# vita-epfl/CrowdNav

Measured on AMD Instinct MI355X. Metric: env-steps/sec (whole node), 4096 envs x 5 humans, ORCA step, higher is better.
Workload: dtype f32 ORCA solve + f64 env step

## Files before the change

### crowdnav_amd/csrc/rollout_fused.h

```cpp
#pragma once
#include "step_kernels.h"

namespace cn {

constexpr int kFusedMaxNC = 5;

template <typename T>
__device__ __forceinline__ T in_vgpr(T x) {
    asm volatile("" : "+v"(x));
    return x;
}

__device__ __forceinline__ void stage_agent(const Params& P, const Smem& s, const Lane& L, const AgentRegs& r,
                                            double human_safety) {
    if (L.lane >= P.nA) return;
    s.kin[L.lane] = make_float4((float)r.px, (float)r.py, (float)r.vx, (float)r.vy);
    s.posd[L.lane] = make_double2(r.px, r.py);
    s.rad[L.lane] = r.rad;
    s.hview[L.lane] = (float)(r.rad + 0.01 + human_safety);
}

__device__ __forceinline__ void preferred_velocity(const AgentRegs& r, float max_speed, bool solve, float4& sol, float4& start) {
    const double gdx = r.gx - r.px, gdy = r.gy - r.py;
    const double speed = norm2(gdx, gdy);
    const float pref_x = (float)(speed > 1.0 ? gdx / speed : gdx);
    const float pref_y = (float)(speed > 1.0 ? gdy / speed : gdy);
    sol = make_float4(pref_x, pref_y, max_speed, solve ? 1.0f : 0.0f);
    float sx, sy;
    lp_start_point(max_speed, pref_x, pref_y, sx, sy);
    start = make_float4(sx, sy, 0.0f, 0.0f);
}

#define CN_FUSED_SYNC() wave_lds_sync()



struct PairRow {
    int my_info, my_slot;
    unsigned long long row_slots;
};
__device__ __forceinline__ PairRow pair_row_of(const Params& P, const Smem& s, int lane) {
    PairRow pr{0, P.nA, 0ull};
    if (lane < P.pairs) {
        pr.my_info = s.pinfo[lane];
        const int c = (pr.my_info >> 16) & 0xff;
        for (int k = 0; k < kFusedMaxNC; ++k) {
            int slot = P.nA;
            if (k < P.NC) {
                const int ik = s.pinfo[lane - c + k];
                slot = ((ik >> 24) & 1) ? ((ik >> 8) & 0xff) : P.nA;
            }
            pr.row_slots |= (unsigned long long)slot << (8 * k);
        }
        pr.my_slot = (int)((pr.row_slots >> (8 * c)) & 0xffull);
    }
    return pr;
}

template <typename Mid>
__device__ __forceinline__ void fused_pair_phase(const Params& P, const Smem& s, const PairRow& pr, float range_sq, Mid&& mid) {
    const int my_info = pr.my_info, my_slot = pr.my_slot;
    const unsigned long long row_slots = pr.row_slots;
    const int q = my_info & 0xff, c = (my_info >> 16) & 0xff;
    const int ol = (my_info >> 8) & 0xff;
    const bool robot_sim = (my_info >> 25) & 1;
    const float4 me = s.kin[q];
    const float4 other = s.kin[my_slot];
    float4 ot[kFusedMaxNC];
#pragma unroll
    for (int k = 0; k < kFusedMaxNC; ++k) ot[k] = s.kin[(int)((row_slots >> (8 * k)) & 0xffull)];
    const float* view = robot_sim ? s.rview : s.hview;
    const float rsum = view[q] + view[ol];
    const float odx = me.x - other.x, ody = me.y - other.y;
    const float mine = odx * odx + ody * ody;
    int rank = 0, within = 0;
    {
        const uint32_t mb = __float_as_uint(mine), rb = __float_as_uint(range_sq);
        uint32_t before = 0u, inside = 0u;
#pragma unroll
        for (int k = 0; k < kFusedMaxNC; ++k) {
            const float dx = me.x - ot[k].x, dy = me.y - ot[k].y;
            const uint32_t vb = __float_as_uint(dx * dx + dy * dy);
            const uint32_t tie = (uint32_t)(k - c) >> 31;
            before = __builtin_amdgcn_alignbit(before, vb - mb - tie, 31);
            inside = __builtin_amdgcn_alignbit(inside, vb - rb, 31);
        }
        within = __popc(inside);
        rank = __popc(before & inside);
    }
    mid();
    if (c == 0) s.count[q] = within < P.orca.max_neighbors ? within : P.orca.max_neighbors;
    if (mine < range_sq && rank < P.orca.max_neighbors)
        s.lines[q * kLineStride + rank] =
            make_half_plane(P.orca, me.x, me.y, me.z, me.w, other.x, other.y, other.z, other.w, rsum);
}

template <int MAXL>
__device__ __forceinline__ void fused_candidates(const Params& P, const Smem& s, int lane) {
    if (lane < P.nA * MAXL) {
        const int q = lane / MAXL, k = lane - q * MAXL;
        const float4 so = s.sol[q];
        const float4* lq = s.lines + q * kLineStride;
        s.cand2[q * kLineStride + k] = lp_line_candidate_pairs5(lq, k, lane, so.z, so.x, so.y);
    }
}

__device__ __forceinline__ void split_barrier() {
    asm volatile("s_waitcnt lgkmcnt(0)\n\ts_barrier" ::: "memory");
}

struct Lp3Item {
    int a, m, i, base;
    bool item;
    float4 li, lj;
    float radius;
};
template <int MAXL>
__device__ __forceinline__ Lp3Item lp3_item_of(const Smem& s, int lane, unsigned long long mask) {
    constexpr int kPairs = MAXL * (MAXL - 1) / 2;
    Lp3Item it;
    const int t = lane / kPairs;
    it.m = lane - t * kPairs;
    it.a = 0;
    unsigned long long rest = mask;
#pragma unroll
    for (int u = 0; u < kWave / kPairs; ++u) {
        const int bit = rest ? __ffsll((long long)rest) - 1 : 0;
        it.a = (u == t) ? bit : it.a;
        rest &= rest - 1ull;
    }
    it.item = lane < (int)__popcll(mask) * kPairs;
    it.i = lp3_program_of(it.m), it.base = it.i * (it.i - 1) / 2;
    const float4* la = s.lines + it.a * kLineStride;
    it.li = la[it.i], it.lj = la[it.m - it.base];
    it.radius = s.sol[it.a].z;
    return it;
}
template <int MAXL>
__device__ __forceinline__ void lp3_head(const Smem& s, const Lp3Item& it) {
    const float4 pr = lp3_project(it.li, it.lj);
    if (it.item) s.proj[it.a * kLineStride + it.m] = pr;
    CN_FUSED_SYNC();
    if (it.item) {
        const float4* pa = s.proj + it.a * kLineStride + it.base;
        s.cand3[it.a * kLineStride + it.m] =
            lp_line_candidate<MAXL - 2>(pa[it.m - it.base], pa, it.m - it.base, it.radius, -it.li.w, it.li.z, true);
    }
}

template <int MAXL>
__device__ __forceinline__ bool split_has_head(unsigned int pred, int u, int n_steps) {
    return pred != 0u && __popc(pred) * (MAXL * (MAXL - 1) / 2) <= kWave && u < n_steps;
}

struct NoOp {
    __device__ __forceinline__ void operator()() const {}
};
template <int MAXL, int BASE_PRIO = 0, typename AfterScan = NoOp>
__device__ __forceinline__ unsigned long long fused_solve(const Params& P, const Smem& s, int lane, bool solve, float& rx,
                                                          float& ry, PhaseClock* clk, unsigned long long have = 0ull,
                                                          AfterScan&& after_scan = NoOp{}) {
    (void)P, (void)clk;
    rx = 0.0f, ry = 0.0f;
    int n = 0, fail = 0;
    if (solve) {
        n = s.count[lane];
        const float4 start = s.res[lane];
        rx = start.x, ry = start.y;
        fail = lp_planar_scan<MAXL>(s.lines + lane * kLineStride, s.cand2 + lane * kLineStride, n, rx, ry);
    }
    CN_TICK(clk, 3);
    const bool need = solve && fail < n;
    const unsigned long long nm = __ballot(need);
#ifdef CN_PHASE_TIMING
    if (clk) clk->acc[9] += __popcll(nm);
#endif
    after_scan();
    if (nm == 0ull) __builtin_amdgcn_s_setprio(BASE_PRIO);
    if (nm != 0ull) {
        __builtin_amdgcn_s_setprio(3);
        constexpr int kPairs = MAXL * (MAXL - 1) / 2;
        const int n_todo = __popcll(nm);
        bool one_pass_done = false;
        if (n_todo * kPairs <= kWave) {
            const Lp3Item it = lp3_item_of<MAXL>(s, lane, nm);
            const bool item = it.item;
            const int a = it.a, i = it.i, m = it.m, base = it.base;
            const float4 li = it.li;
            const float radius = it.radius;
            const bool hit = (nm & ~have) == 0ull;
            if (!hit) {
                lp3_head<MAXL>(s, it);
                CN_FUSED_SYNC();
            }
            if (item && m == base)
                s.cand2[a * kLineStride + i] = lp3_inner_program(s.proj + a * kLineStride, s.cand3 + a * kLineStride, i, li, radius);
            CN_FUSED_SYNC();
            if (need)
                lp3_outer_scan(s.lines + lane * kLineStride, s.cand2 + lane * kLineStride, n, fail, s.sol[lane].z, rx, ry);
            one_pass_done = true;
        } else {
            if (need) s.todo[__popcll(nm & ((1ull << lane) - 1ull))] = lane;
            CN_FUSED_SYNC();
            const int items = n_todo * kPairs;
            for (int p = lane; p < items; p += kWave) {
                const int t = p / kPairs, m = p - t * kPairs;
                const int a = s.todo[t];
                const int i = lp3_program_of(m), j = m - i * (i - 1) / 2;
                const float4* la = s.lines + a * kLineStride;
                s.proj[a * kLineStride + m] = lp3_project(la[i], la[j]);
            }
            CN_FUSED_SYNC();
            for (int p = lane; p < items; p += kWave) {
                const int t = p / kPairs, m = p - t * kPairs;
                const int a = s.todo[t];
                const int i = lp3_program_of(m), base = i * (i - 1) / 2;
                const float4 li = s.lines[a * kLineStride + i];
                const float4* pa = s.proj + a * kLineStride + base;
                s.cand3[a * kLineStride + m] = lp_line_candidate<MAXL - 2>(pa[m - base], pa, m - base, s.sol[a].z, -li.w, li.z, true);
            }
            CN_FUSED_SYNC();
        }
        if (need && !one_pass_done)
            lp3_scan(s.lines + lane * kLineStride, s.proj + lane * kLineStride, s.cand3 + lane * kLineStride, n,
                     fail, s.sol[lane].z, rx, ry);
    }
    return nm;
}

struct StepConsts {
    double dt, limit, limit1, success, collision, ddist, dfactor, hsafety;
};
__device__ __forceinline__ StepConsts step_consts(const Params& P) {
    StepConsts K;
    K.dt = in_vgpr(P.dt), K.limit = in_vgpr(P.time_limit), K.limit1 = in_vgpr(P.time_limit - 1.0);
    K.success = in_vgpr(P.success_reward), K.collision = in_vgpr(P.collision_penalty);
    K.ddist = in_vgpr(P.discomfort_dist), K.dfactor = in_vgpr(P.discomfort_factor);
    K.hsafety = in_vgpr(P.human_safety);
    return K;
}

__device__ __forceinline__ double swept_distance(const AgentRegs& r, bool human, double2 rp, double act_x, double act_y,
                                                 double new_vx, double new_vy, double dt, double robot_rad) {
    const double x1 = r.px - rp.x, y1 = r.py - rp.y;
    const double wx = r.vx - act_x, wy = r.vy - act_y;
    const double x2 = x1 + wx * dt, y2 = y1 + wy * dt;
    const double sx = x2 - x1, sy = y2 - y1;
    double u = ((0.0 - x1) * sx + (0.0 - y1) * sy) / (sx * sx + sy * sy);
    u = (u > 1.0) ? 1.0 : ((u < 0.0) ? 0.0 : u);
    const bool degenerate = (sx == 0.0 && sy == 0.0);
    const double cx = degenerate ? 0.0 - x1 : (x1 + u * sx) - 0.0;
    const double cy = degenerate ? 0.0 - y1 : (y1 + u * sy) - 0.0;
    const double endx = r.px + new_vx * dt, endy = r.py + new_vy * dt;
    const double d = norm2(human ? cx : endx - r.gx, human ? cy : endy - r.gy);
    return human ? d - r.rad - robot_rad : d;
}

struct StepOutcome {
    double reward, dmin;
    int info;
    bool done;
};
__device__ __forceinline__ StepOutcome reduce_env(const Params& P, const Smem& s, int ebase, double gtime, const StepConsts& K) {
    const double goal_dist = s.closest[ebase];
    const double robot_rad = s.rad[ebase];
    double dmin = std::numeric_limits<double>::infinity();
    bool collision = false;
    for (int i = 1; i < P.A; ++i) {
        const double c = s.closest[ebase + i];
        const bool hit = c < 0.0;
        dmin = (!collision & !hit & (c < dmin)) ? c : dmin;
        collision = collision | hit;
    }
    const bool timeout = gtime >= K.limit1;
    const bool reaching = goal_dist < robot_rad;
    const bool danger = dmin < K.ddist;
    double reward = danger ? (dmin - K.ddist) * K.dfactor * K.dt : 0.0;
    int info = danger ? CN_DANGER : CN_NOTHING;
    reward = reaching ? K.success : reward, info = reaching ? CN_REACH_GOAL : info;
    reward = collision ? K.collision : reward, info = collision ? CN_COLLISION : info;
    reward = timeout ? 0.0 : reward, info = timeout ? CN_TIMEOUT : info;
    const bool done = timeout | collision | reaching;
    return StepOutcome{reward, dmin, info, done};
}


#ifdef CN_WAVE_TRACE
static __device__ unsigned long long cn_wave_trace[8192 * 6];
#endif

constexpr int kSplitOrcaPrio = 1;
constexpr int kAssistHead = 1;
#ifndef CN_SPLIT_HEAD_PRIO
#define CN_SPLIT_HEAD_PRIO 2
#endif
#ifndef CN_SPLIT_HEAD_TAIL_PRIO
#define CN_SPLIT_HEAD_TAIL_PRIO 1
#endif

#ifdef CN_SPLIT_PROBE
constexpr bool kSplitProbe = true;
static __device__ unsigned long long cn_split_probe[32];
#define SPLIT_PROBE_DECL()                                                                                   \
    unsigned long long sp_cnt[7] = {}, sp_wait[3] = {}, sp_w1[2] = {}, sp_n1[2] = {}, sp_dt = 0ull; \
    bool sp_prev_head = false
#define SPLIT_PROBE_WAIT(k, barrier)                                   \
    do {                                                               \
        const unsigned long long sp_t0 = __builtin_readcyclecounter(); \
        barrier;                                                       \
        sp_dt = __builtin_readcyclecounter() - sp_t0;                  \
        sp_wait[k] += sp_dt;                                           \
    } while (0)
#define SPLIT_PROBE_AFTER_1(word, head)                               \
    do {                                                               \
        if ((word) != 0u) sp_w1[0] += sp_dt, ++sp_n1[0];               \
        if (sp_prev_head) sp_w1[1] += sp_dt, ++sp_n1[1];               \
        sp_prev_head = (head);                                         \
    } while (0)
#define SPLIT_PROBE_STEP(ended, nm, head, pred)                                  \
    do {                                                                         \
        const bool sp_hit = (head) && (nm) != 0ull && ((nm) & ~(unsigned long long)(pred)) == 0ull; \
        ++sp_cnt[0], sp_cnt[1] += (ended) ? 1 : 0, sp_cnt[2] += (nm) != 0ull ? 1 : 0, sp_cnt[3] += (head) ? 1 : 0; \
        sp_cnt[4] += sp_hit ? 1 : 0, sp_cnt[5] += ((nm) != 0ull && !sp_hit) ? 1 : 0, sp_cnt[6] += ((head) && (nm) == 0ull) ? 1 : 0; \
    } while (0)
#define SPLIT_PROBE_FLUSH(lane, base)                                                        \
    do {                                                                                     \
        if ((lane) == 0) {                                                                   \
            if ((base) == 0)                                                                 \
                for (int k = 0; k < 7; ++k) atomicAdd(&cn_split_probe[k], sp_cnt[k]);        \
            for (int k = 0; k < 3; ++k) atomicAdd(&cn_split_probe[((base) ? 10 : 7) + k], sp_wait[k]); \
            for (int k = 0; k < 2; ++k) {                                                    \
                atomicAdd(&cn_split_probe[((base) ? 17 : 13) + k], sp_w1[k]);                \
                atomicAdd(&cn_split_probe[((base) ? 19 : 15) + k], sp_n1[k]);                \
            }                                                                                \
        }                                                                                    \
    } while (0)
#else
constexpr bool kSplitProbe = false;
#define SPLIT_PROBE_DECL() (void)0
#define SPLIT_PROBE_WAIT(k, barrier) barrier
#define SPLIT_PROBE_AFTER_1(word, head) (void)0
#define SPLIT_PROBE_STEP(ended, nm, head, pred) (void)0
#define SPLIT_PROBE_FLUSH(lane, base) (void)0
#endif

template <int MAXL, int ASSIST>
__device__ __forceinline__ void split_orca_wave(const Params& P, const Smem& s, int n_steps) {
    const int lane = (int)threadIdx.x - kWave;
    float2* const vel = reinterpret_cast<float2*>(s.act);
    const float range_sq = P.orca.neighbor_dist * P.orca.neighbor_dist;
    const double c_dt = in_vgpr(P.dt);
    split_barrier();
    __builtin_amdgcn_s_setprio(kSplitOrcaPrio);
    const PairRow pr = pair_row_of(P, s, lane);
    double px = 0.0, py = 0.0;
    float rx = 0.0f, ry = 0.0f;
    bool solved = false;
    SPLIT_PROBE_DECL();
    for (int u = 0;;) {
        SPLIT_PROBE_WAIT(0, split_barrier());
        const bool ended = __builtin_amdgcn_readfirstlane(s.flag[0]) != 0;
        const unsigned int pred = ((ASSIST & kAssistHead) || kSplitProbe) ? (unsigned int)__builtin_amdgcn_readfirstlane(s.flag[1]) : 0u;
        if (!ended) ++u;
        if (u >= n_steps) {
            split_barrier();
            break;
        }
        const bool head = (ASSIST & kAssistHead) ? split_has_head<MAXL>(pred, u, n_steps) : false;
        SPLIT_PROBE_AFTER_1(pred, head);
        if (lane < P.nA) {
            if (ended) {
                const double2 p = s.posd[lane];
                px = p.x, py = p.y;
            } else if (solved) {
                px = px + (double)rx * c_dt;
                py = py + (double)ry * c_dt;
                s.kin[lane] = make_float4((float)px, (float)py, rx, ry);
            }
        }
        CN_FUSED_SYNC();
        if (lane < P.pairs) fused_pair_phase(P, s, pr, range_sq, [] {});
        SPLIT_PROBE_WAIT(1, split_barrier());
        fused_candidates<MAXL>(P, s, lane);
        CN_FUSED_SYNC();
        solved = lane < P.nA && s.sol[lane < P.nA ? lane : 0].w != 0.0f;
        const unsigned long long nm = fused_solve<MAXL, kSplitOrcaPrio>(P, s, lane, solved, rx, ry, nullptr, head ? pred : 0u, [&] {
            if (head) SPLIT_PROBE_WAIT(2, split_barrier());
        });
        if (lane < P.nA) vel[lane] = make_float2(rx, ry);
        if (((ASSIST & kAssistHead) || kSplitProbe) && lane == 0) s.flag[1] = (int)nm;
        SPLIT_PROBE_STEP(ended, nm, head, pred);
    }
    SPLIT_PROBE_FLUSH(lane, 0);
}

template <bool HEADLINE, bool SPLIT = false, int ASSIST = 0>
__global__ __launch_bounds__((SPLIT ? 2 : 1) * kWave, (SPLIT ? 4 : HEADLINE ? 3 : 1)) void rollout_fused_kernel(
    Params P_in, const StateView* Sd, const int* ring_filled_in, RolloutView R, int n_steps, const double* ext_action) {
    static_assert(HEADLINE || !SPLIT, "the two-wave kernel exists for the headline geometry only");
    static_assert(SPLIT || ASSIST == 0, "the env wave assists an ORCA wave: two-wave kernel only");
#ifdef CN_WAVE_TRACE
    const unsigned long long wt_entry = __builtin_amdgcn_s_memrealtime();
    unsigned long long wt_fallbacks = 0ull, wt_ends = 0ull;
#endif
    constexpr int MAXL = 5;
    Params P = P_in;
    P.async_fill = 0;
    if (HEADLINE) {
        P.A = 6, P.NC = 5, P.E = 2, P.nA = 12, P.pairs = 60, P.threads = 64;
    }
    const Smem s = carve<MAXL>(P);
    if constexpr (SPLIT) {
        if (__builtin_amdgcn_readfirstlane((int)threadIdx.x) >= kWave) {
            split_orca_wave<MAXL, ASSIST>(P, s, n_steps);
            return;
        }
    }
    const Lane L = lane_of(P);
    AgentRegs r = {};
    float robot_max_speed = 0.0f;
    const bool robot = L.valid && L.a == 0;
    const cn_rollout_io* iop = R.io;
    double theta = 0.0;
    EpisodeBook ep = {};
    {
        const StateView S = *Sd;
        const cn_rollout_io io = *iop;
        const size_t gi = L.valid ? L.gi : 0;
        const int env = L.valid ? L.env : 0;
        const double2 p0 = S.pos[gi], v0 = S.vel[gi], g0 = S.goal[gi], q0 = S.rv[gi];
        const bool have = P.robot_orca ? S.rsim_valid[env] != 0 : false;
        const float rr_kept = P.robot_orca ? S.rsim_radius[gi] : 0.0f;
        const float ms_kept = P.robot_orca ? S.rsim_max_speed[env] : 0.0f;
        const double theta0 = S.theta[env];
        EpisodeBook ep0;
        CN_LOAD_EPISODE(ep0, S, io, ring_filled_in, env);
        if (L.valid) {
            r.px = p0.x, r.py = p0.y, r.vx = v0.x, r.vy = v0.y, r.gx = g0.x, r.gy = g0.y, r.rad = q0.x, r.vpref = q0.y;
            ep = ep0;
            if (L.a == 0) theta = theta0;
            if (P.robot_orca) {
                const float rr = have ? rr_kept : (float)(r.rad + 0.01 + P.robot_safety);
                if (!have) S.rsim_radius[L.gi] = rr;
                s.rview[L.lane] = rr;
                if (L.a == 0) {
                    robot_max_speed = have ? ms_kept : (float)r.vpref;
                    if (!have) S.rsim_max_speed[L.env] = robot_max_speed;
                }
            }
        }
    }
    build_pairs(P, s);

    if (L.valid && ep.state == kWaitingScenario && scenario_ready(P, *Sd, L.env, ep.ep_count, ep.ring_filled)) {
        load_from_ring(P, *Sd, L, ep.ep_count % P.ring_depth, r);
        ep.state = kRunning;
        ep.gtime = 0.0;
        theta = 1.5707963267948966;
    }
    unsigned int transitions = 0;
    for (int t = threadIdx.x; t < kMaxDiscount; t += P.threads) s.disc[t] = t < R.discount_len ? R.discount[t] : 0.0;
    CN_FUSED_SYNC();
    if (L.lane == 0) s.kin[P.nA] = make_float4(std::numeric_limits<float>::infinity(), std::numeric_limits<float>::infinity(), 0.0f, 0.0f);
    const PairRow pr = pair_row_of(P, s, L.lane);
    const StepConsts K = step_consts(P);
    stage_agent(P, s, L, r, K.hsafety);
    CN_FUSED_SYNC();

#ifdef CN_PHASE_TIMING
    PhaseClock clock = {};
    PhaseClock* clk = &clock;
    clock.last = __builtin_readcyclecounter();
#else
    PhaseClock* clk = nullptr;
    (void)clk;
#endif
    const float range_sq = P.orca.neighbor_dist * P.orca.neighbor_dist;
#ifdef CN_WAVE_TRACE
    const unsigned long long wt_loop = __builtin_amdgcn_s_memrealtime();
#endif
    if constexpr (SPLIT) {
        float2* const vel = reinterpret_cast<float2*>(s.act);
        if (L.lane == 0) s.flag[0] = 1, s.flag[1] = 0;
        split_barrier();
        bool skip = true;
        SPLIT_PROBE_DECL();
        for (int u = 0;;) {
            SPLIT_PROBE_WAIT(0, split_barrier());
            if (!skip) ++u;
            const unsigned int pred = ((ASSIST & kAssistHead) || kSplitProbe) ? (unsigned int)__builtin_amdgcn_readfirstlane(s.flag[1]) : 0u;
            SPLIT_PROBE_AFTER_1(pred, (ASSIST & kAssistHead) != 0 && split_has_head<MAXL>(pred, u, n_steps));
            const bool running = L.valid && ep.state == kRunning;
            const AgentRegs r0 = r;
            double act_x = 0.0, act_y = 0.0, new_vx = 0.0, new_vy = 0.0;
            if (!skip && L.lane < P.nA) {
                const float2 mine = vel[L.lane], robots = vel[L.ebase];
                act_x = (double)robots.x, act_y = (double)robots.y;
                new_vx = (L.a == 0) ? act_x : (double)mine.x;
                new_vy = (L.a == 0) ? act_y : (double)mine.y;
                if (running) {
                    r.px = r.px + new_vx * K.dt;
                    r.py = r.py + new_vy * K.dt;
                    r.vx = new_vx;
                    r.vy = new_vy;
                }
            }
            if (u < n_steps && L.lane < P.nA) {
                float4 sol4, start4;
                preferred_velocity(r, (L.a == 0) ? robot_max_speed : (float)r.vpref, running && (L.a > 0 || P.robot_orca), sol4, start4);
                s.sol[L.lane] = sol4;
                s.res[L.lane] = start4;
            }
            SPLIT_PROBE_WAIT(1, split_barrier());
            if constexpr ((ASSIST & kAssistHead) != 0) {
                if (split_has_head<MAXL>(pred, u, n_steps)) {
                    __builtin_amdgcn_s_setprio(CN_SPLIT_HEAD_PRIO);
                    const Lp3Item it = lp3_item_of<MAXL>(s, L.lane, (unsigned long long)pred);
                    lp3_head<MAXL>(s, it);
                    __builtin_amdgcn_s_setprio(CN_SPLIT_HEAD_TAIL_PRIO);
                    SPLIT_PROBE_WAIT(2, split_barrier());
                }
            }
            bool ended = false;
            if (!skip) {
                const double2 rp = make_double2(__shfl(r0.px, L.ebase), __shfl(r0.py, L.ebase));
                if (L.valid) s.closest[L.lane] = swept_distance(r0, L.a > 0, rp, act_x, act_y, new_vx, new_vy, K.dt, s.rad[L.ebase]);
                CN_FUSED_SYNC();
                bool done = false;
                if (running) {
                    const double disc_t = s.disc[ep.cur_steps < kMaxDiscount ? ep.cur_steps : kMaxDiscount - 1];
                    const StepOutcome o = reduce_env(P, s, L.ebase, ep.gtime, K);
                    done = o.done;
                    ep.gtime += K.dt;
                    ++transitions;
                    CN_BOOK_TRANSITION(ep, ep.cur_steps < kMaxDiscount ? disc_t : 0.0, o.reward, o.info, o.dmin);
                    if (done) {
                        const cn_rollout_io io = *iop;
                        const StateView S = *Sd;
                        AgentRegs next = r;
                        load_from_ring(P, S, L, (ep.ep_count + 1) % P.ring_depth, next);
                        CN_END_EPISODE(P, S, io, L.env, L.a == 0, K.limit, o.info, ep, r = next; theta = 1.5707963267948966);
                    }
                }
                ended = __ballot(done) != 0ull;
            }
            if (ended) stage_agent(P, s, L, r, K.hsafety);
            if (L.lane == 0) s.flag[0] = ended ? 1 : 0;
            skip = ended;
            if constexpr ((ASSIST & kAssistHead) != 0 && CN_SPLIT_HEAD_TAIL_PRIO != 0) __builtin_amdgcn_s_setprio(0);
            if (u >= n_steps) break;
        }
        SPLIT_PROBE_FLUSH(L.lane, 10);
    }
    const int one_wave_steps = SPLIT ? 0 : n_steps;
    for (int step = 0; step < one_wave_steps; ++step) {
        const bool running = L.valid && ep.state == kRunning;
        const bool solve = running && (L.a > 0 || P.robot_orca);

        if (L.lane < P.pairs) {
            float4 sol4, start4;
            fused_pair_phase(P, s, pr, range_sq, [&] {
                preferred_velocity(r, (L.a == 0) ? robot_max_speed : (float)r.vpref, solve, sol4, start4);
            });
            if (L.lane < P.nA) {
                s.sol[L.lane] = sol4;
                s.res[L.lane] = start4;
            }
        }
        CN_FUSED_SYNC();
        CN_TICK(clk, 2);

        fused_candidates<MAXL>(P, s, L.lane);
        CN_FUSED_SYNC();

        float rx, ry;
        const bool fell_back = fused_solve<MAXL>(P, s, L.lane, solve, rx, ry, clk) != 0ull;
        (void)fell_back;
#ifdef CN_WAVE_TRACE
        if (fell_back) ++wt_fallbacks;
#endif
        CN_TICK(clk, 8);

        double act_x, act_y;
        if (P.robot_orca) {
            act_x = (double)__shfl(rx, L.ebase);
            act_y = (double)__shfl(ry, L.ebase);
        } else {
            act_x = L.valid ? ext_action[2 * (size_t)L.env] : 0.0;
            act_y = L.valid ? ext_action[2 * (size_t)L.env + 1] : 0.0;
        }
        const double new_vx = (L.a == 0) ? act_x : (double)rx;
        const double new_vy = (L.a == 0) ? act_y : (double)ry;

        if (L.valid)
            s.closest[L.lane] = swept_distance(r, L.a > 0, s.posd[L.ebase], act_x, act_y, new_vx, new_vy, K.dt, s.rad[L.ebase]);
        CN_FUSED_SYNC();
        CN_TICK(clk, 5);

        if (running) {
            const double disc_t = s.disc[ep.cur_steps < kMaxDiscount ? ep.cur_steps : kMaxDiscount - 1];
            const StepOutcome o = reduce_env(P, s, L.ebase, ep.gtime, K);
            const double reward = o.reward, dmin = o.dmin;
            const int info = o.info;
            const bool done = o.done;
            ep.gtime += K.dt;
            r.px = r.px + new_vx * K.dt;
            r.py = r.py + new_vy * K.dt;
            r.vx = new_vx;
            r.vy = new_vy;
            ++transitions;
            CN_BOOK_TRANSITION(ep, ep.cur_steps < kMaxDiscount ? disc_t : 0.0, reward, info, dmin);
#ifdef CN_WAVE_TRACE
            if (__ballot(done) != 0ull) ++wt_ends;
#endif
            if (done) {
                const cn_rollout_io io = *iop;
                CN_END_EPISODE(P, *Sd, io, L.env, L.a == 0, K.limit, info, ep,
                               load_from_ring(P, *Sd, L, ep.ep_count % P.ring_depth, r); theta = 1.5707963267948966);
            }
        }
        stage_agent(P, s, L, r, K.hsafety);
        CN_FUSED_SYNC();
        CN_TICK(clk, 7);
    }
#ifdef CN_PHASE_TIMING
    if ((threadIdx.x & (kWave - 1)) == 0) {
        unsigned long long total = 0ull;
        for (int k = 0; k < 10; ++k) {
            atomicAdd(&cn_phase_cycles[k], clock.acc[k]);
            if (k != 9) total += clock.acc[k];
        }
        atomicMax(&cn_phase_cycles[14], total);
        atomicMin(&cn_phase_cycles[13], total);
        atomicAdd(&cn_phase_cycles[15], 1ull);
    }
#endif

#ifdef CN_WAVE_TRACE
    const unsigned long long wt_exit = __builtin_amdgcn_s_memrealtime();
#endif
    const StateView S = *Sd;
    if (L.valid) CN_STORE_AGENT(S, L.gi, r);
    const cn_rollout_io io = *iop;
    if (robot) CN_STORE_EPISODE(P, S, io, L.env, ep, theta);
    rollout_epilogue(P, S, io, L, robot, transitions, ep.ep_count, reinterpret_cast<double*>(s.lines));
#ifdef CN_WAVE_TRACE
    if (threadIdx.x == 0 && blockIdx.x < 8192) {
        unsigned long long* w = cn_wave_trace + 6 * blockIdx.x;
        unsigned hw;
        asm volatile("s_getreg_b32 %0, hwreg(HW_REG_HW_ID)" : "=s"(hw));
        w[0] = wt_entry, w[1] = wt_loop, w[2] = wt_exit, w[3] = __builtin_amdgcn_s_memrealtime();
        w[4] = wt_fallbacks | (wt_ends << 32), w[5] = hw;
    }
#endif
}

}
```

Before: 1.425 billion.

## Track per-agent episode end and step budget in split-wave control word

Replaces the single wave-wide 'ended' flag and shared step counter with a bitmask word holding, per agent lane, whether its position must be reread and whether it still needs further steps. The ORCA helper wave now decides termination and the LP3 head assist from this word, and the head runs only for agents that did not just reset. Envs whose episode ended no longer force every agent into a skipped iteration. This is meant to reduce wasted lockstep iterations across the whole wave, at the cost of extra ballots and mask logic in each iteration.

```diff
diff --git a/crowdnav_amd/csrc/rollout_fused.h b/crowdnav_amd/csrc/rollout_fused.h
--- a/crowdnav_amd/csrc/rollout_fused.h
+++ b/crowdnav_amd/csrc/rollout_fused.h
@@ -148,9 +148,16 @@
     }
 }
 
+__device__ __forceinline__ unsigned int split_word(unsigned long long reread, unsigned long long needs, int nA) {
+    const unsigned int agents = (1u << nA) - 1u;
+    return ((unsigned int)reread & agents) | (((unsigned int)needs & agents) << 16);
+}
+__device__ __forceinline__ bool split_last_iteration(unsigned int word) { return (word >> 16) == 0u; }
+__device__ __forceinline__ bool split_reread(unsigned int word, int agent_lane) { return ((word >> agent_lane) & 1u) != 0u; }
 template <int MAXL>
-__device__ __forceinline__ bool split_has_head(unsigned int pred, int u, int n_steps) {
-    return pred != 0u && __popc(pred) * (MAXL * (MAXL - 1) / 2) <= kWave && u < n_steps;
+__device__ __forceinline__ unsigned int split_head_agents(unsigned int pred, unsigned int word) {
+    const unsigned int agents = pred & ~word & (word >> 16);
+    return (agents != 0u && __popc(agents) * (MAXL * (MAXL - 1) / 2) <= kWave) ? agents : 0u;
 }
 
 struct NoOp {
@@ -302,7 +309,7 @@
 constexpr bool kSplitProbe = true;
 static __device__ unsigned long long cn_split_probe[32];
 #define SPLIT_PROBE_DECL()                                                                                   \
-    unsigned long long sp_cnt[7] = {}, sp_wait[3] = {}, sp_w1[2] = {}, sp_n1[2] = {}, sp_dt = 0ull; \
+    unsigned long long sp_cnt[9] = {}, sp_wait[3] = {}, sp_w1[2] = {}, sp_n1[2] = {}, sp_dt = 0ull; \
     bool sp_prev_head = false
 #define SPLIT_PROBE_WAIT(k, barrier)                                   \
     do {                                                               \
@@ -317,17 +324,19 @@
         if (sp_prev_head) sp_w1[1] += sp_dt, ++sp_n1[1];               \
         sp_prev_head = (head);                                         \
     } while (0)
-#define SPLIT_PROBE_STEP(ended, nm, head, pred)                                  \
+#define SPLIT_PROBE_STEP(word, robots, nm, head, pred)                           \
     do {                                                                         \
         const bool sp_hit = (head) && (nm) != 0ull && ((nm) & ~(unsigned long long)(pred)) == 0ull; \
-        ++sp_cnt[0], sp_cnt[1] += (ended) ? 1 : 0, sp_cnt[2] += (nm) != 0ull ? 1 : 0, sp_cnt[3] += (head) ? 1 : 0; \
+        const unsigned int sp_need = ((word) >> 16) & (robots);                  \
+        ++sp_cnt[0], sp_cnt[1] += ((word) & sp_need) != 0u ? 1 : 0, sp_cnt[2] += (nm) != 0ull ? 1 : 0, sp_cnt[3] += (head) ? 1 : 0; \
         sp_cnt[4] += sp_hit ? 1 : 0, sp_cnt[5] += ((nm) != 0ull && !sp_hit) ? 1 : 0, sp_cnt[6] += ((head) && (nm) == 0ull) ? 1 : 0; \
+        sp_cnt[7] += __popc((word) & sp_need), sp_cnt[8] += __popc((robots) & ~sp_need);                  \
     } while (0)
 #define SPLIT_PROBE_FLUSH(lane, base)                                                        \
     do {                                                                                     \
         if ((lane) == 0) {                                                                   \
             if ((base) == 0)                                                                 \
-                for (int k = 0; k < 7; ++k) atomicAdd(&cn_split_probe[k], sp_cnt[k]);        \
+                for (int k = 0; k < 9; ++k) atomicAdd(&cn_split_probe[k < 7 ? k : k + 14], sp_cnt[k]); \
             for (int k = 0; k < 3; ++k) atomicAdd(&cn_split_probe[((base) ? 10 : 7) + k], sp_wait[k]); \
             for (int k = 0; k < 2; ++k) {                                                    \
                 atomicAdd(&cn_split_probe[((base) ? 17 : 13) + k], sp_w1[k]);                \
@@ -340,12 +349,12 @@
 #define SPLIT_PROBE_DECL() (void)0
 #define SPLIT_PROBE_WAIT(k, barrier) barrier
 #define SPLIT_PROBE_AFTER_1(word, head) (void)0
-#define SPLIT_PROBE_STEP(ended, nm, head, pred) (void)0
+#define SPLIT_PROBE_STEP(word, robots, nm, head, pred) (void)0
 #define SPLIT_PROBE_FLUSH(lane, base) (void)0
 #endif
 
 template <int MAXL, int ASSIST>
-__device__ __forceinline__ void split_orca_wave(const Params& P, const Smem& s, int n_steps) {
+__device__ __forceinline__ void split_orca_wave(const Params& P, const Smem& s) {
     const int lane = (int)threadIdx.x - kWave;
     float2* const vel = reinterpret_cast<float2*>(s.act);
     const float range_sq = P.orca.neighbor_dist * P.orca.neighbor_dist;
@@ -357,19 +366,18 @@
     float rx = 0.0f, ry = 0.0f;
     bool solved = false;
     SPLIT_PROBE_DECL();
-    for (int u = 0;;) {
+    for (;;) {
         SPLIT_PROBE_WAIT(0, split_barrier());
-        const bool ended = __builtin_amdgcn_readfirstlane(s.flag[0]) != 0;
+        const unsigned int word = (unsigned int)__builtin_amdgcn_readfirstlane(s.flag[0]);
         const unsigned int pred = ((ASSIST & kAssistHead) || kSplitProbe) ? (unsigned int)__builtin_amdgcn_readfirstlane(s.flag[1]) : 0u;
-        if (!ended) ++u;
-        if (u >= n_steps) {
+        if (split_last_iteration(word)) {
             split_barrier();
             break;
         }
-        const bool head = (ASSIST & kAssistHead) ? split_has_head<MAXL>(pred, u, n_steps) : false;
-        SPLIT_PROBE_AFTER_1(pred, head);
+        const unsigned int head = (ASSIST & kAssistHead) ? split_head_agents<MAXL>(pred, word) : 0u;
+        SPLIT_PROBE_AFTER_1(pred, head != 0u);
         if (lane < P.nA) {
-            if (ended) {
+            if (split_reread(word, lane)) {
                 const double2 p = s.posd[lane];
                 px = p.x, py = p.y;
             } else if (solved) {
@@ -384,12 +392,12 @@
         fused_candidates<MAXL>(P, s, lane);
         CN_FUSED_SYNC();
         solved = lane < P.nA && s.sol[lane < P.nA ? lane : 0].w != 0.0f;
-        const unsigned long long nm = fused_solve<MAXL, kSplitOrcaPrio>(P, s, lane, solved, rx, ry, nullptr, head ? pred : 0u, [&] {
+        const unsigned long long nm = fused_solve<MAXL, kSplitOrcaPrio>(P, s, lane, solved, rx, ry, nullptr, head, [&] {
             if (head) SPLIT_PROBE_WAIT(2, split_barrier());
         });
         if (lane < P.nA) vel[lane] = make_float2(rx, ry);
         if (((ASSIST & kAssistHead) || kSplitProbe) && lane == 0) s.flag[1] = (int)nm;
-        SPLIT_PROBE_STEP(ended, nm, head, pred);
+        SPLIT_PROBE_STEP(word, 1u | (1u << P.A), nm, head != 0u, head);
     }
     SPLIT_PROBE_FLUSH(lane, 0);
 }
@@ -412,7 +420,7 @@
     const Smem s = carve<MAXL>(P);
     if constexpr (SPLIT) {
         if (__builtin_amdgcn_readfirstlane((int)threadIdx.x) >= kWave) {
-            split_orca_wave<MAXL, ASSIST>(P, s, n_steps);
+            split_orca_wave<MAXL, ASSIST>(P, s);
             return;
         }
     }
@@ -481,15 +489,19 @@
 #endif
     if constexpr (SPLIT) {
         float2* const vel = reinterpret_cast<float2*>(s.act);
-        if (L.lane == 0) s.flag[0] = 1, s.flag[1] = 0;
+        if (L.lane == 0) s.flag[0] = (int)split_word(~0ull, n_steps > 0 ? ~0ull : 0ull, P.nA), s.flag[1] = 0;
         split_barrier();
         bool skip = true;
+        int u = 0;
         SPLIT_PROBE_DECL();
-        for (int u = 0;;) {
+        for (;;) {
             SPLIT_PROBE_WAIT(0, split_barrier());
+            const unsigned int word = (unsigned int)__builtin_amdgcn_readfirstlane(s.flag[0]);
+            const unsigned int pred = ((ASSIST & kAssistHead) || kSplitProbe) ? (unsigned int)__builtin_amdgcn_readfirstlane(s.flag[1]) : 0u;
+            const bool last = split_last_iteration(word);
+            const unsigned int head = (ASSIST & kAssistHead) ? split_head_agents<MAXL>(pred, word) : 0u;
+            SPLIT_PROBE_AFTER_1(pred, head != 0u);
             if (!skip) ++u;
-            const unsigned int pred = ((ASSIST & kAssistHead) || kSplitProbe) ? (unsigned int)__builtin_amdgcn_readfirstlane(s.flag[1]) : 0u;
-            SPLIT_PROBE_AFTER_1(pred, (ASSIST & kAssistHead) != 0 && split_has_head<MAXL>(pred, u, n_steps));
             const bool running = L.valid && ep.state == kRunning;
             const AgentRegs r0 = r;
             double act_x = 0.0, act_y = 0.0, new_vx = 0.0, new_vy = 0.0;
@@ -505,28 +517,32 @@
                     r.vy = new_vy;
                 }
             }
-            if (u < n_steps && L.lane < P.nA) {
+            if (!last && L.lane < P.nA) {
                 float4 sol4, start4;
-                preferred_velocity(r, (L.a == 0) ? robot_max_speed : (float)r.vpref, running && (L.a > 0 || P.robot_orca), sol4, start4);
+                preferred_velocity(r, (L.a == 0) ? robot_max_speed : (float)r.vpref,
+                                   running && u < n_steps && (L.a > 0 || P.robot_orca), sol4, start4);
                 s.sol[L.lane] = sol4;
                 s.res[L.lane] = start4;
             }
             SPLIT_PROBE_WAIT(1, split_barrier());
             if constexpr ((ASSIST & kAssistHead) != 0) {
-                if (split_has_head<MAXL>(pred, u, n_steps)) {
+                if (head != 0u) {
                     __builtin_amdgcn_s_setprio(CN_SPLIT_HEAD_PRIO);
-                    const Lp3Item it = lp3_item_of<MAXL>(s, L.lane, (unsigned long long)pred);
+                    const Lp3Item it = lp3_item_of<MAXL>(s, L.lane, (unsigned long long)head);
                     lp3_head<MAXL>(s, it);
                     __builtin_amdgcn_s_setprio(CN_SPLIT_HEAD_TAIL_PRIO);
                     SPLIT_PROBE_WAIT(2, split_barrier());
                 }
             }
-            bool ended = false;
+            const bool finished = u >= n_steps;
+            const unsigned int agents = (1u << P.nA) - 1u;
+            const unsigned int may_end = (unsigned int)__ballot(!finished) & agents;
+            const unsigned int word_advancing = ((unsigned int)__ballot(u + 1 < n_steps) & agents) << 16;
+            bool done = false;
+            const double2 rp = make_double2(__shfl(r0.px, L.ebase), __shfl(r0.py, L.ebase));
             if (!skip) {
-                const double2 rp = make_double2(__shfl(r0.px, L.ebase), __shfl(r0.py, L.ebase));
                 if (L.valid) s.closest[L.lane] = swept_distance(r0, L.a > 0, rp, act_x, act_y, new_vx, new_vy, K.dt, s.rad[L.ebase]);
                 CN_FUSED_SYNC();
-                bool done = false;
                 if (running) {
                     const double disc_t = s.disc[ep.cur_steps < kMaxDiscount ? ep.cur_steps : kMaxDiscount - 1];
                     const StepOutcome o = reduce_env(P, s, L.ebase, ep.gtime, K);
@@ -542,13 +558,14 @@
                         CN_END_EPISODE(P, S, io, L.env, L.a == 0, K.limit, o.info, ep, r = next; theta = 1.5707963267948966);
                     }
                 }
-                ended = __ballot(done) != 0ull;
-            }
+            }
+            const bool ended = done && !finished;
             if (ended) stage_agent(P, s, L, r, K.hsafety);
-            if (L.lane == 0) s.flag[0] = ended ? 1 : 0;
-            skip = ended;
+            skip = ended || finished;
+            const unsigned int ends = (unsigned int)__ballot(done) & may_end;
+            if (L.lane == 0) s.flag[0] = (int)(split_word(ends, ends, P.nA) | word_advancing);
             if constexpr ((ASSIST & kAssistHead) != 0 && CN_SPLIT_HEAD_TAIL_PRIO != 0) __builtin_amdgcn_s_setprio(0);
-            if (u >= n_steps) break;
+            if (last) break;
         }
         SPLIT_PROBE_FLUSH(L.lane, 10);
     }
```

Result: no change. 1.421 billion (-0.3%).
